# dobraczka/kiez

Hardware: AMD Instinct MI355X
Metric: source queries/sec (fit+kneighbors) + recall@k vs reference, 1/2/4/8 GPU (higher is better)
Workload: dtype f16

## Files before the change

### include/kiez_amd.h

```cpp
#ifndef KIEZ_AMD_H
#define KIEZ_AMD_H

#include <stddef.h>
#include <stdint.h>

#ifdef __cplusplus
extern "C" {
#endif

#define KZ_ABI_VERSION 7
#define KZ_MAX_CANDIDATES 4096
#define KZ_MERGE_MAX_ENTRIES 8192

enum { KZ_OK = 0, KZ_ERR_INVALID = 1, KZ_ERR_HIP = 2, KZ_ERR_UNSUPPORTED = 3, KZ_ERR_NOMEM = 4, KZ_ERR_NONFINITE = 5 };
enum { KZ_F32 = 0, KZ_F64 = 1 };
enum { KZ_EUCLIDEAN = 0, KZ_SQEUCLIDEAN = 1, KZ_COSINE = 2, KZ_MANHATTAN = 3, KZ_CHEBYSHEV = 4, KZ_MINKOWSKI = 5,
       KZ_BRAYCURTIS = 6, KZ_SEUCLIDEAN = 7, KZ_CORRELATION = 8, KZ_HAMMING = 9,
       KZ_JACCARD = 10, KZ_DICE = 11, KZ_ROGERSTANIMOTO = 12, KZ_RUSSELLRAO = 13, KZ_SOKALMICHENER = 14, KZ_SOKALSNEATH = 15,
       KZ_YULE = 16 };

typedef struct kz_ctx kz_ctx;
typedef struct kz_matrix kz_matrix;

typedef struct kz_knn_stats {
// ... 6 lines not shown
    int32_t n_blocks;
    int32_t first_pass;
    int64_t n_escalated_rows;
    double max_err_ratio;
    int32_t dual;
    int32_t n_first_pass_fail;
    int64_t n_events;
    int64_t n_overflow_rows;
    int64_t n_logged_groups;
    int32_t wide_lists;
    int32_t n_spec_rows;
    double probe_ms;
    int64_t n_range_rows;
    int64_t n_range_pairs;
    int64_t n_range_group_rows;
} kz_knn_stats;

int kz_abi_version(void);
const char* kz_last_error(void);
int kz_device_count(int* n);
int kz_ctx_create(int device, void* stream, kz_ctx** out);
int kz_ctx_destroy(kz_ctx* ctx);
int kz_ctx_sync(kz_ctx* ctx);
int kz_ctx_trim(kz_ctx* ctx);
int kz_ctx_set_option(kz_ctx* ctx, const char* name, double value);

int kz_malloc(kz_ctx* ctx, size_t bytes, void** d_ptr);
int kz_free(kz_ctx* ctx, void* d_ptr);
int kz_memcpy_h2d(kz_ctx* ctx, void* d_dst, const void* h_src, size_t bytes);
int kz_memcpy_d2h(kz_ctx* ctx, void* h_dst, const void* d_src, size_t bytes);
// ... 90 lines not shown
```

### kiez_amd/_native.py

```python
from __future__ import annotations

import ctypes as C
import os
import sys
import threading
from pathlib import Path
from typing import Optional, Tuple

import numpy as np

_LIB_NAME = "libkiez_amd.so"
_lib = None
_lock = threading.Lock()

KZ_F32, KZ_F64 = 0, 1
KZ_EUCLIDEAN, KZ_SQEUCLIDEAN, KZ_COSINE, KZ_MANHATTAN, KZ_CHEBYSHEV, KZ_MINKOWSKI = 0, 1, 2, 3, 4, 5
KZ_BRAYCURTIS, KZ_SEUCLIDEAN, KZ_CORRELATION, KZ_HAMMING = 6, 7, 8, 9
KZ_JACCARD, KZ_DICE, KZ_ROGERSTANIMOTO, KZ_RUSSELLRAO, KZ_SOKALMICHENER, KZ_SOKALSNEATH, KZ_YULE = 10, 11, 12, 13, 14, 15, 16
BOOLEAN_METRICS = ("jaccard", "dice", "rogerstanimoto", "russellrao", "sokalmichener", "sokalsneath", "yule")
METRIC_IDS = {"euclidean": KZ_EUCLIDEAN, "sqeuclidean": KZ_SQEUCLIDEAN, "cosine": KZ_COSINE, "manhattan": KZ_MANHATTAN,
              "chebyshev": KZ_CHEBYSHEV, "minkowski": KZ_MINKOWSKI, "braycurtis": KZ_BRAYCURTIS, "seuclidean": KZ_SEUCLIDEAN,
              "correlation": KZ_CORRELATION, "hamming": KZ_HAMMING, "jaccard": KZ_JACCARD, "dice": KZ_DICE,
              "rogerstanimoto": KZ_ROGERSTANIMOTO, "russellrao": KZ_RUSSELLRAO, "sokalmichener": KZ_SOKALMICHENER,
              "sokalsneath": KZ_SOKALSNEATH, "yule": KZ_YULE}
# ... 23 lines not shown
        ("n_blocks", C.c_int32),
        ("first_pass", C.c_int32),
        ("n_escalated_rows", C.c_int64),
        ("max_err_ratio", C.c_double),
        ("dual", C.c_int32),
        ("n_first_pass_fail", C.c_int32),
        ("n_events", C.c_int64),
        ("n_overflow_rows", C.c_int64),
        ("n_logged_groups", C.c_int64),
        ("wide_lists", C.c_int32),
        ("n_spec_rows", C.c_int32),
        ("probe_ms", C.c_double),
        ("n_range_rows", C.c_int64),
        ("n_range_pairs", C.c_int64),
        ("n_range_group_rows", C.c_int64),
    ]

    def as_dict(self):
        return {name: getattr(self, name) for name, _ in self._fields_}


_P = C.c_void_p
_I64 = C.c_int64
SYMBOLS = [
    ("kz_abi_version", C.c_int, []),
    ("kz_last_error", C.c_char_p, []),
    ("kz_device_count", C.c_int, [C.POINTER(C.c_int)]),
    ("kz_ctx_create", C.c_int, [C.c_int, _P, C.POINTER(_P)]),
    ("kz_ctx_destroy", C.c_int, [_P]),
    ("kz_ctx_sync", C.c_int, [_P]),
# ... 375 lines not shown
```

### kiez_amd/csrc/kz_common.h

```cpp
#pragma once
#include <hip/hip_runtime.h>

#include <cstdarg>
#include <cstdint>
#include <cstdio>
#include <cstring>
#include <memory>

#include "../../include/kiez_amd.h"
#include "kz_pool_buf.h"

#define KZ_TILE 128
#define KZ_KSLICE 16
#define KZ_LIVE_MAX 1024
#define KZ_POOL_SLOTS 256

constexpr double KZ_K_NESTED_MIN_MS = 2.0;
constexpr int KZ_K_DUAL_SHORT_DIV = 5;
constexpr int KZ_K_DUAL_SHORT_KP = 16;
constexpr double KZ_K_PROBE_MIN_MS = 12.0;
constexpr int KZ_K_EXACT_DIRECT_ROWS = 32;
constexpr double KZ_K_SPEC_ELEMS = 1.6e9;
constexpr int KZ_K_FLOOR_PROBE = 1024;

struct kz_ctx {
    int device;
    hipStream_t stream;
    bool own_stream;
    hipEvent_t ev[12];
    int stream2_busy;
    hipStream_t stream2;
    double eps_scale;
    int force_splits;
    int chunk_rows;
    int precision;
    int dual_stride;
    int esc_bf;
    int short_ord_min_tiles;
// ... 8 lines not shown
    int dual_force;
    int h_q64;
    int fin_fast_div;
    double probe_min_pairs;
    int list_floor;
    int tier_probe;
    int dual_nested;
    int esc_ladder;
    int exact_rows;
    int abl;
    double floor_margin;
    int dual_rank;
    int spec_rows;
    int wide_lists;
    int wide_sel;
    void* scratch;
    size_t scratch_bytes;
    float* floor_buf;
    size_t floor_bytes;
    int* d_counters;
    int* h_counters;
    int n_cus;
    void* h_stage;
    size_t h_stage_bytes;
    int h_stage_flip;
    struct { void* ptr; size_t bytes; } pool[KZ_POOL_SLOTS];
    int pool_n;
    size_t pool_bytes;
    void* live_ptr[KZ_LIVE_MAX];
    size_t live_bytes[KZ_LIVE_MAX];
// ... 320 lines not shown
```

### kiez_amd/csrc/kz_floor.h

```cpp
#pragma once

static inline bool kz_floor_fit(const double* pairs, int n_probe, double margin_scale, double* model) {
    model[0] = model[1] = model[2] = 0.0;
    if (n_probe <= 0) return false;
    double sx = 0, sy = 0;
    for (int i = 0; i < n_probe; ++i) {
        sx += pairs[2 * i];
        sy += pairs[2 * i + 1];
    }
    const double mx = sx / n_probe, my = sy / n_probe;
    double sxx = 0, sxy = 0;
    for (int i = 0; i < n_probe; ++i) {
        sxx += (pairs[2 * i] - mx) * (pairs[2 * i] - mx);
        sxy += (pairs[2 * i] - mx) * (pairs[2 * i + 1] - my);
    }
    const double beta = sxx > 0 ? sxy / sxx : 0.0, alpha = my - beta * mx;
    double short_max = 0;
    for (int i = 0; i < n_probe; ++i) {
        const double r = alpha + beta * pairs[2 * i] - pairs[2 * i + 1];
        if (r > short_max) short_max = r;
    }
    model[0] = alpha;
    model[1] = beta;
    model[2] = short_max * margin_scale;
    return (alpha - alpha == 0.0) && (beta - beta == 0.0) && (model[2] - model[2] == 0.0);
}
```

### kiez_amd/csrc/kz_knn.hip

```cpp
#include <vector>

#include <algorithm>
#include <atomic>
#include <type_traits>

#include "kz_common.h"
#include "kz_bool.h"
#include "kz_floor.h"

#include "kz_knn_device.h"

template <int KP, int NRES>
__global__ __launch_bounds__(256, 3) void kz_knn_cand_kernel(KnnCandParams p) {
    extern __shared__ __attribute__((aligned(16))) char smem[];
    float* ybuf = reinterpret_cast<float*>(smem);
    const int tid = threadIdx.x;
    const int lane = tid & 63;
    const int wave = tid >> 6;
    const int j = lane & 31;
    const int h = lane >> 5;

    const int4 wd = p.work[blockIdx.x];
    const int qt = wd.x;
    const int t_begin = wd.y;
// ... 348 lines not shown
        return;
    }
    const double qc2 = rowq[r * 3 + 0], qh = rowq[r * 3 + 1], qr = rowq[r * 3 + 2];
    const double Yh = y_hmax[0], Ry = y_hmax[1], Yc2 = y_hmax[2];
    const double qc = sqrt(qc2), yc = sqrt(Yc2);
    const double eps = eps_mult * (qr * Yh + qh * Ry + qr * Ry + gamma_acc * (0.5 * Yc2 + qh * Yh) +
                                   1.1920928955078125e-07 * (qc + yc) * (qc + yc) + 1e-12 * (0.5 * Yc2 + qc2));
    const double f = (alpha + beta * qc2 - margin - eps) / hscale[1];
    float ff = (float)f;
    if ((double)ff > f) ff = nextafterf(ff, -INFINITY);
    out[p] = ff;
}

static inline double kz_gamma_acc_h(int kg) { return 2.0 * (double)(kg * 4 + 16) * 5.9604644775390625e-08; }
static int kz_floor_model(kz_ctx* ctx, const double* dist, const double* rowq, int n_probe, int64_t stride, int k, int metric, double* model,
                          bool* ok) {
    KzPoolBuf<double> d_pairs;
    int rc = d_pairs.alloc(ctx, (size_t)n_probe * 16);
    if (rc != KZ_OK) return rc;
    std::vector<double> hp((size_t)n_probe * 2);
    hipLaunchKernelGGL(kz_floor_pairs_kernel, dim3((unsigned)((n_probe + 255) / 256)), dim3(256), 0, ctx->stream, dist, rowq, n_probe, stride, k,
                       metric, d_pairs.get());
    hipError_t e = hipGetLastError();
    if (e == hipSuccess) e = hipMemcpyAsync(hp.data(), d_pairs.get(), (size_t)n_probe * 16, hipMemcpyDeviceToHost, ctx->stream);
    if (e == hipSuccess) e = hipStreamSynchronize(ctx->stream);
    d_pairs.reset();
    if (e != hipSuccess) {
        kz_set_error("kz_knn: floor probe failed: %s", hipGetErrorString(e));
        return KZ_ERR_HIP;
    }
    *ok = kz_floor_fit(hp.data(), n_probe, ctx->floor_margin, model);
    return KZ_OK;
}

__global__ void kz_boot_floor_kernel(const float* __restrict__ in_key, const int* __restrict__ in_idx, KzListLayout lay, int KP, int64_t list_row0,
                                     int64_t q_begin, int64_t q_count, const float* __restrict__ prev, float* __restrict__ out) {
    const int64_t q = (int64_t)blockIdx.x * blockDim.x + threadIdx.x;
    if (q >= q_count) return;
    const int64_t l0 = kz_list_contig_off(list_row0 + q, lay, KP, 0);
    float mn = INFINITY;
    bool full = true;
    for (int e = 0; e < KP; ++e) {
        full = full && in_idx[l0 + e] >= 0;
        mn = fminf(mn, in_key[l0 + e]);
    }
    float f = full ? mn : -INFINITY;
// ... 120 lines not shown
    KZ_REQUIRE(query->ctx == ctx && index->ctx == ctx, "%s: matrices belong to a different context", who);
    KZ_REQUIRE(!query->raw_only && !index->raw_only, "%s: a rows-only matrix (kz_matrix_create rows_on_device = 3) cannot be searched", who);
    KZ_REQUIRE(query->d == index->d, "%s: feature dimensions differ (%lld vs %lld)", who, (long long)query->d, (long long)index->d);
    KZ_REQUIRE(query->dtype == index->dtype, "%s: query and index must have the same dtype", who);
    KZ_REQUIRE(query->metric == index->metric && query->mink_p == index->mink_p, "%s: query and index were packed for different metrics", who);
    KZ_REQUIRE(kz_metric_params_match(query, index), "%s: seuclidean needs the same V (kz_matrix_set_seuclidean_v) on query and index", who);
    KZ_REQUIRE(q_begin >= 0 && q_count >= 0 && q_begin + q_count <= query->n, "%s: query row range out of bounds", who);
    return KZ_OK;
}

static int kz_knn_impl(kz_ctx* ctx, kz_matrix* query, int64_t q_begin, int64_t q_count, kz_matrix* index, int k,
                       int exclude_self, const int64_t* d_self_ids, KzResearch rs, double* d_dist,
                       int64_t* d_ind, kz_knn_stats* stats, KzDualPass* dual);
static int kz_escalate_rows(kz_ctx* ctx, kz_matrix* query, int64_t cq_begin, const int* fail_list, int n_fail, kz_matrix* index, int k,
                            int exclude_self, const int64_t* d_self_ids, KzResearch rs, double* out_dist,
                            int64_t* out_ind, kz_knn_stats* st2, float* ms_out) {
    KZ_HIP(hipEventRecord(ctx->ev[3], ctx->stream));
    const size_t row_bytes = (size_t)query->d * (query->dtype == KZ_F32 ? 4 : 8);
    KzPoolBuf<int64_t> sub_ind;
    KzPoolBuf<double> sub_dist;
    KzPoolBuf<int64_t> sub_self;
    KzPoolBuf<void> sub_raw;
    KzPoolBuf<int> fl;
    KzMatrixPtr qsub;
    int rc = fl.alloc(ctx, (size_t)n_fail * sizeof(int));
    if (rc == KZ_OK) rc = sub_raw.alloc(ctx, (size_t)n_fail * row_bytes);
    if (rc == KZ_OK && exclude_self) rc = sub_self.alloc(ctx, (size_t)n_fail * 8);
    if (rc == KZ_OK) rc = sub_dist.alloc(ctx, (size_t)n_fail * k * 8);
    if (rc == KZ_OK) rc = sub_ind.alloc(ctx, (size_t)n_fail * k * 8);
    if (rc != KZ_OK) return rc;
    hipError_t e = hipMemcpyAsync(fl.get(), fail_list, (size_t)n_fail * sizeof(int), hipMemcpyDeviceToDevice, ctx->stream);
// ... 2 lines not shown
                           n_fail, (int64_t)row_bytes, (char*)sub_raw.get(), sub_self.get(), d_self_ids);
        e = hipGetLastError();
    }
    if (e != hipSuccess) {
        kz_set_error("kz_knn: gathering the escalated rows failed: %s", hipGetErrorString(e));
        return KZ_ERR_HIP;
    }
    kz_matrix* qsub_new = nullptr;
    rc = kz_matrix_create(ctx, sub_raw.get(), 2, n_fail, query->d, query->dtype, query->metric, &qsub_new);
    qsub.reset(qsub_new);
    memset(st2, 0, sizeof(*st2));
    if (rc == KZ_OK)
        rc = kz_knn_impl(ctx, qsub.get(), 0, n_fail, index, k, exclude_self, sub_self.get(), rs, sub_dist.get(), sub_ind.get(), st2, nullptr);
    if (rc == KZ_OK) {
        hipLaunchKernelGGL(kz_scatter_rows_kernel, dim3((unsigned)(((int64_t)n_fail * k + 255) / 256)), dim3(256), 0, ctx->stream,
                           sub_dist.get(), sub_ind.get(), fl.get(), n_fail, k, out_dist, out_ind);
        e = hipGetLastError();
        if (e == hipSuccess) e = hipEventRecord(ctx->ev[4], ctx->stream);
        if (e == hipSuccess) e = hipStreamSynchronize(ctx->stream);
        if (e != hipSuccess) {
            kz_set_error("kz_knn: scattering the escalated rows failed: %s", hipGetErrorString(e));
            rc = KZ_ERR_HIP;
        }
    }
    if (rc != KZ_OK) return rc;
    KZ_HIP(hipEventElapsedTime(ms_out, ctx->ev[3], ctx->ev[4]));
    return KZ_OK;
}

__global__ void kz_strided_pick_kernel(const int* __restrict__ in, int n_out, int64_t stride, int* __restrict__ out) {
    const int i = blockIdx.x * blockDim.x + threadIdx.x;
// ... 673 lines not shown
```

### kiez_amd/csrc/kz_knn_dual.h

```cpp
#pragma once

constexpr int KZ_EVC = 1;

__global__ __launch_bounds__(256) void kz_dual_theta_kernel(const float* __restrict__ in_key, const int* __restrict__ in_idx,
                                                            KzListLayout lay, int KP, int rank, int64_t n_b, int64_t n_b_pad,
                                                            const float* __restrict__ bias_b, const double* __restrict__ a_hmax,
                                                            const double* __restrict__ b_hmax, const double* __restrict__ hscale,
                                                            float* __restrict__ theta, float* __restrict__ floor_,
                                                            const int* __restrict__ idx_to_row, int sev_cap, int* __restrict__ sev_cnt,
                                                            uint2* __restrict__ sev) {
    const int lane = threadIdx.x & 63;
    const int64_t t = (int64_t)blockIdx.x * 4 + (threadIdx.x >> 6);
    if (t >= n_b_pad) return;
    if (t >= n_b) {
        if (lane == 0) theta[t] = INFINITY;
        return;
    }
    const int M = lay.pieces[kz_list_region(t, lay)] * KP;
    const int64_t l0 = kz_list_contig_off(t, lay, KP, 0);
    float x[4];
    int valid[4];
    unsigned ux[4];
    unsigned all_or = 0u, all_and = 0xffffffffu;
    int nv = 0;
// ... 49 lines not shown
                if (pos < sev_cap) sev[t * (int64_t)sev_cap + pos] = make_uint2(__float_as_uint(x[u]), (unsigned)idx_to_row[in_idx[l0 + lane + 64 * u]]);
            }
            base += (int)__popcll(mask);
        }
        if (lane == 0) sev_cnt[t] = base;
    }
    if (lane == 0) {
        const double S2 = hscale[0] * hscale[0];
        const double margin = 4.76837158203125e-07 * S2 * (a_hmax[0] * b_hmax[0] + a_hmax[2] + b_hmax[2]);
        const double th = (double)tau + (double)bias_b[t] - margin;
        float tf = (float)th;
        if ((double)tf > th) tf = nextafterf(tf, -INFINITY);
        theta[t] = tf;
        floor_[t] = tau_bound;
    }
}

__global__ __launch_bounds__(256) void kz_dual_sample_kernel(const uint4* __restrict__ packed, const float* __restrict__ bias,
                                                             int nsr, int stride, int s_tiles, int P,
                                                             uint4* __restrict__ s_packed, float* __restrict__ s_bias) {
    const int jp = blockIdx.x;
    const int n_frag = 2 * nsr * KZ_TILE;
    for (int e = threadIdx.x; e < n_frag; e += 256) {
        const int row = e & (KZ_TILE - 1), blk = e >> 7;
        const int64_t j = kz_dealt_row((int64_t)jp * KZ_TILE + row, (int64_t)s_tiles * KZ_TILE, P);
        const int64_t src_tile = (j >> 7) * stride;
        s_packed[(int64_t)jp * n_frag + e] = packed[src_tile * n_frag + blk * KZ_TILE + (j & (KZ_TILE - 1))];
        if (blk == 0) s_bias[(int64_t)jp * KZ_TILE + row] = bias[src_tile * KZ_TILE + (j & (KZ_TILE - 1))];
    }
}
// ... 451 lines not shown
        const double img_b = ((double)s_tiles + (double)a_tiles + (double)b_tiles) * (double)n_slices * 4096.0;
        size_t free_b = 0, total_b = 0;
        KZ_HIP(hipMemGetInfo(&free_b, &total_b));
        const double avail = (double)free_b + (double)ctx->pool_bytes - 2.0 * (double)(1ull << 30);
        const double budget = ctx->dual_max_gb > 0 ? ctx->dual_max_gb * (double)(1ull << 30) : KZ_DUAL_MAX_BYTES;
        if (ev_b + log_b + img_b > budget || ev_b + log_b + img_b > avail)
            return kz_knn_dual_separately(ctx, a, b, k, d_dist_ab, d_ind_ab, d_dist_ba, d_ind_ba, stats_ab, stats_ba);
    }

    int rc = kz_himage_ensure(a, b);
    if (rc != KZ_OK) return rc;
    const kz_himage* ia = a->himg;
    const kz_himage* ib = b->himg;
    const int64_t b_pad = b_tiles * KZ_TILE, a_pad = a_tiles * KZ_TILE;

    const int ev_cap = (int)(((int64_t)rank * stride + (int64_t)(7.0 * sqrt((double)rank) * stride) + 63) & ~(int64_t)63);
    const long long log_cap = (long long)((double)b->n * rank * stride * 1.5) + (1 << 20);

    int then = 0, sep_prec = -1, sep_wide = 0;
    kz_knn_stats st_ba;
    memset(&st_ba, 0, sizeof(st_ba));
    const int rc_pass = [&]() -> int {
    KzPoolBuf<unsigned long long> d_cnt;
    KzPoolBuf<void> log_meta, log_keys;
    KzPoolBuf<uint2> ev;
    KzPoolBuf<int> fail_list, col_idx, ev_cnt;
    KzPoolBuf<float> col_key, qfloor, qnb, floor_, theta;
    KzPoolBuf<int> perm, iota;
    KzPoolBuf<float> theta_min, theta_s;
    KzPoolBuf<int> row_map, q_sorted, q_iota;
    KzPoolBuf<float> q_key_s, q_key, q_bias;
    KzPoolBuf<unsigned short> q_packed;
    KzPoolBuf<float> p_bias;
    KzPoolBuf<unsigned short> p_packed;
// ... 26 lines not shown
    if (rc == KZ_OK) rc = q_iota.alloc(ctx, (size_t)a_pad * 4);
    if (rc == KZ_OK) rc = q_sorted.alloc(ctx, (size_t)a_pad * 4);
    if (rc == KZ_OK) rc = row_map.alloc(ctx, (size_t)a_pad * 4);
    if (rc == KZ_OK) rc = p_bias.alloc(ctx, (size_t)b_pad * 4);
    if (rc == KZ_OK) rc = theta_s.alloc(ctx, (size_t)b_pad * 4);
    if (rc == KZ_OK) rc = theta_min.alloc(ctx, (size_t)b_pad * 4);
    if (rc == KZ_OK) rc = iota.alloc(ctx, (size_t)b_pad * 4);
    if (rc == KZ_OK) rc = perm.alloc(ctx, (size_t)b_pad * 4);
    if (rc == KZ_OK) rc = theta.alloc(ctx, (size_t)b_pad * 4);
    if (rc == KZ_OK) rc = floor_.alloc(ctx, (size_t)b_pad * 4);
    if (rc == KZ_OK) rc = qnb.alloc(ctx, (size_t)a_pad * 4);
    if (rc == KZ_OK) rc = col_key.alloc(ctx, (size_t)b->n * KPr * 4);
    if (rc == KZ_OK) rc = col_idx.alloc(ctx, (size_t)b->n * KPr * 4);
    if (rc == KZ_OK) rc = ev_cnt.alloc(ctx, (size_t)b_pad * 4 * KZ_EVC);
    if (rc == KZ_OK) rc = fail_list.alloc(ctx, (size_t)b->n * 4);
    if (rc == KZ_OK) rc = ev.alloc(ctx, (size_t)b_pad * ev_cap * 8);
    if (rc == KZ_OK) rc = log_keys.alloc(ctx, (size_t)log_cap * 16);
    if (rc == KZ_OK) rc = log_meta.alloc(ctx, (size_t)log_cap * 8);
    if (rc == KZ_OK) rc = d_cnt.alloc(ctx, KZ_DUAL_CNT_BYTES);
    if (rc != KZ_OK) {
        then = 1;
        return KZ_OK;
    }
    double floor_model[3] = {0, 0, 0};
    bool have_floor = false;
    bool tier_probed = false;
    bool want_floor = ctx->list_floor && KZ_K_FLOOR_PROBE > 0 && a->n >= (int64_t)16 * KZ_K_FLOOR_PROBE &&
                      (ctx->dual_force || t_sweep_ms >= (KP > 16 ? 12.0 : 25.0));
    const bool want_tier = !ctx->dual_force && ctx->tier_probe > 0 && ctx->esc_bf && a->n >= (int64_t)16 * ctx->tier_probe &&
                           ((double)a->n * (double)b->n >= ctx->probe_min_pairs || t_sweep_ms >= KZ_K_PROBE_MIN_MS);
    if (want_tier && ctx->list_floor && KZ_K_FLOOR_PROBE > 0 && a->n >= (int64_t)16 * KZ_K_FLOOR_PROBE) want_floor = true;
    if (want_floor || want_tier) {
        const int n_probe = want_floor ? KZ_K_FLOOR_PROBE : (ctx->tier_probe < 1024 ? ctx->tier_probe : 1024);
        const int64_t pstride = a->n / n_probe;
        KzPoolBuf<int> plist;
        rc = plist.alloc(ctx, (size_t)n_probe * sizeof(int));
        if (rc == KZ_OK && want_floor) rc = qfloor.alloc(ctx, (size_t)a_pad * 4);
        kz_knn_stats stp;
        memset(&stp, 0, sizeof(stp));
// ... 14 lines not shown
                rc = kz_escalate_rows(ctx, a, 0, plist.get(), n_probe, b, k, 0, nullptr, kz_research_wide(ctx->wide_lists), d_dist_ab, d_ind_ab, &stw,
                                      &wms);
                if (rc == KZ_OK && stw.wide_lists > 0 && (int64_t)stw.n_first_pass_fail * 4 <= n_probe &&
                    (int64_t)stw.n_first_pass_fail * 2 < stp.n_first_pass_fail)
                    wide = ctx->wide_lists;
            }
            if (rc != KZ_OK) return rc;
            if (wide > 0 || (int64_t)stp.n_first_pass_fail * 2 > n_probe) {
                then = 1;
                sep_prec = wide > 0 ? -1 : 2;
                sep_wide = wide;
                return KZ_OK;
            }
        }
        plist.reset();
        if (rc == KZ_OK && want_floor) rc = kz_floor_model(ctx, d_dist_ab, ia->rowq, n_probe, pstride, k, a->metric, floor_model, &have_floor);
        if (rc != KZ_OK) return rc;
        if (!have_floor) qfloor.reset();
    }

    auto sample_lists = [&](int rank_, int64_t tiles_, int* kps_out, int* force_out, int head = 2) {
        int kps = KP, force = 0;
        if (ctx->dual_sample_short && KP > 16) {
            kps = rank_ > 96 ? 32 : 16;
            const int need = (head * rank_ + kps - 1) / kps, cap = 256 / kps;
            force = need < cap ? need : cap;
            if ((int64_t)force * 4 > tiles_ || force * kps < rank_) {
                kps = KP;
                force = 0;
            }
        }
        *kps_out = kps;
        *force_out = force;
// ... 6 lines not shown
    hipLaunchKernelGGL(kz_dual_c2key_kernel, dim3((unsigned)((a->n + 255) / 256)), dim3(256), 0, ctx->stream, ia->rowq, a->n, q_key.get());
    hipLaunchKernelGGL(kz_iota_kernel, dim3((unsigned)((a_pad + 255) / 256)), dim3(256), 0, ctx->stream, q_iota.get(), (int)a_pad);
    KZ_HIP(hipGetLastError());
    rc = kz_sort_pairs_f32_i32(ctx, q_key.get(), q_key_s.get(), q_iota.get(), q_sorted.get(), (int)a->n, 0);
    if (rc != KZ_OK) return rc;
    hipLaunchKernelGGL(kz_dual_deal_kernel, dim3((unsigned)((a_pad + 255) / 256)), dim3(256), 0, ctx->stream, q_sorted.get(), a->n, a_pad, row_map.get());
    KZ_HIP(hipGetLastError());
    rc = kz_himage_pack_permuted(a, row_map.get(), q_packed.get(), q_bias.get());
    if (rc != KZ_OK) return rc;
    hipLaunchKernelGGL(kz_dual_negbias_kernel, dim3((unsigned)((a_pad + 255) / 256)), dim3(256), 0, ctx->stream, q_bias.get(), a->n, a_pad, qnb.get());

    int rank3 = 0, stride3 = 0, KPs3 = KP, force_s3 = 0, ev_cap3 = 0;
    int64_t s3_tiles = 0;
    long long log_cap3 = 0;
    const int64_t s_img_rows = s_tiles * KZ_TILE;
    bool nested = ctx->dual_nested && s_tiles >= 8 && s_tiles < a->n / KZ_TILE && s_img_rows >= (int64_t)8 * KP &&
                  b->n <= kz_rows_per_chunk(ctx, KP, false) && (ctx->dual_force || t_sweep_ms / stride >= KZ_K_NESTED_MIN_MS);
    if (nested) {
        const double t2_ms = 2.0 * (double)b->n * (double)s_img_rows * (double)(a->kg * 4) / 1e12;
        const int rank3_safe = k + 1 < KP ? k + 1 : KP;
        rank3 = rank3_safe;
        if (ctx->dual_rank > 0)
            rank3 = ctx->dual_rank < rank3_safe ? ctx->dual_rank : rank3_safe;
        else if (ctx->dual_rank == 0 && t2_ms >= 4.0)
            rank3 = kz_dual_pick_rank(k, rank3_safe, t2_ms, (double)b->n, (double)s_img_rows);
        const double s_opt = sqrt(t2_ms / ((double)s_img_rows * rank3 * 0.20e-6));
        stride3 = s_opt < 4.0 ? 4 : (s_opt > 32.0 ? 32 : (int)(s_opt + 0.5));
        const int s_max = (int)(4096.0 / ((double)rank3 + 7.0 * sqrt((double)rank3) + 1.0));
        if (stride3 > s_max) stride3 = s_max;
        s3_tiles = (b_tiles + stride3 - 1) / stride3;
        int64_t s3_rows = s3_tiles * KZ_TILE;
        if ((b_tiles - 1) % stride3 == 0) s3_rows -= b_tiles * KZ_TILE - b->n;
// ... 154 lines not shown
            hipLaunchKernelGGL(kz_dual_theta_kernel, dim3((unsigned)((h.b_pad + 3) / 4)), dim3(256), 0, ctx->stream, d2.lists_key, d2.lists_idx,
                               d2.lists_lay, d2.lists_KP, h.rank, h.b_n, h.b_pad, h.ib->bias, h.ia->d_max, h.ib->d_max, h.ib->center->d_scale,
                               h.theta, h.floor_, h.rm3, h.sev_cap, h.sev_cnt, h.sev);
            KZ_HIP(hipGetLastError());
            return kz_dual_enqueue_chain(*h.rv3);
        };
        kz_knn_stats st2;
        ctx->stream2_busy = 1;
        rc = kz_knn_impl(ctx, b, 0, b->n, a, k, 0, nullptr, KzResearch(), d_dist_ba, d_ind_ba, &st2, &dp2);
        if (rc != KZ_OK) return rc;
        if (dp2.broken || !dp2.post_called) {
            then = 1;
            return KZ_OK;
        }
        nested_sweep_ms = st2.main_kernel_ms;
    } else {
        hipLaunchKernelGGL(kz_dual_sample_kernel, dim3((unsigned)s_tiles), dim3(256), 0, ctx->stream, (const uint4*)ia->packed, ia->bias,
                           n_slices, stride, (int)s_tiles, force_s > 0 ? force_s : 1, (uint4*)s_packed.get(), s_bias.get());
        KZ_HIP(hipGetLastError());
        const int KP = KPs;
        int blocks_per_cu = 1;
        KZ_DISPATCH_KP(rc, kz_h_occupancy, (n_slices, &blocks_per_cu));
        if (rc != KZ_OK) return rc;
        KzPass ps;
        const int slots = kz_h_slots(n_slices, blocks_per_cu, ctx->n_cus);
        KzPlan pl;
        kz_plan_tier_pass(ctx, (int)b_tiles, (int)s_tiles, slots, 256 / KP, KP, KZ_TIER_H, 1, force_s, 0, &pl);
        rc = kz_prepare_pass(ctx, pl, (int)s_tiles, slots, KZ_TIER_H, 0, &ps);
        if (rc != KZ_OK) return rc;
        KnnCandParams cp;
// ... 96 lines not shown
    if (rc == KZ_OK && !ctx->dual_overlap && !dp.broken) {
        dp.post_called = 1;
        rc = enqueue_reverse(&rv);
    }
    {
        const hipError_t e2 = hipStreamSynchronize(ctx->stream2);
        ctx->stream2_busy = 0;
        if (rc == KZ_OK && e2 != hipSuccess) {
            kz_set_error("kz_knn_dual: second stream failed: %s", hipGetErrorString(e2));
            rc = KZ_ERR_HIP;
        }
    }
    if (rc != KZ_OK) return rc;
    KZ_HIP(hipEventElapsedTime(&sample_ms, ctx->ev[5], ctx->ev[6]));
    st_ab.dual = 1;
    st_ab.main_kernel_ms += nested_sweep_ms;
    if (nested) {
        int n_fail3 = ctx->h_counters[24];
        unsigned long long hc3[4];
        memcpy(hc3, ctx->h_counters + 28, 32);
        const int* list3 = nst.fail3.get();
        if (hc3[0] > (unsigned long long)log_cap3) {
            n_fail3 = (int)s_img_rows;
            list3 = nst.rm3.get();
        }
        const bool rescued3 = hc3[0] <= (unsigned long long)log_cap3 && spec_s3.R > 0 && n_fail3 > 0 && n_fail3 <= spec_s3.R;
        if (rescued3) {
            st_ab.n_fallback_rows += n_fail3;
            st_ab.n_spec_rows += n_fail3;
        } else if (n_fail3 > 0) {
// ... 10 lines not shown
        double r3;
        memcpy(&r3, ctx->h_counters + 26, 8);
        if (r3 > st_ab.max_err_ratio) st_ab.max_err_ratio = r3;
        st_ab.n_first_pass_fail += n_fail3;
    }
    kz_dual_fill_stats(stats_ab, st_ab);

    if (!dp.broken && !dp.post_called) dp.broken = 1;
    if (!dp.broken) {
        const int n_fail = ctx->h_counters[12];
        unsigned long long hc[4];
        memcpy(hc, ctx->h_counters + 16, 32);
        memcpy(&st_ba.max_err_ratio, ctx->h_counters + 14, 8);
        float ms = 0;
        KZ_HIP(hipEventElapsedTime(&ms, ctx->ev[8], ctx->ev[9]));
        st_ba.main_kernel_ms = sample_ms - (float)nested_sweep_ms + ms;
        KZ_HIP(hipEventElapsedTime(&ms, ctx->ev[9], ctx->ev[10]));
        st_ba.finalize_ms = ms;
        st_ba.list_len = KPr;
        st_ba.n_splits = 1;
        st_ba.first_pass = KZ_TIER_H;
        st_ba.dual = 1;
        st_ba.n_events = (int64_t)hc[1];
        st_ba.n_overflow_rows = (int64_t)hc[2];
        st_ba.n_logged_groups = (int64_t)(hc[0] & ((1ull << 62) - 1));
        if (hc[0] > (unsigned long long)log_cap) {
            dp.broken = 1;
        } else if (spec_ba.R > 0 && n_fail > 0 && n_fail <= spec_ba.R) {
            st_ba.n_fallback_rows = n_fail;
            st_ba.n_spec_rows = n_fail;
        } else if (n_fail > 0) {
// ... 26 lines not shown
```

### kiez_amd/csrc/kz_options.h

```cpp
#pragma once
#include <cstddef>

#include "kz_common.h"

enum { KZ_OPT_INT = 0, KZ_OPT_BOOL = 1, KZ_OPT_F64 = 2 };
enum { KZ_OPT_PUBLIC = 1, KZ_OPT_SET = 2  };

struct KzOption {
    const char* name;
    int kind;
    size_t offset;
    double lo, hi;
    double dflt;
    unsigned flags;
    double allowed[4];
    int n_allowed;
    const char* doc;
};

#define KZ_O(field) offsetof(kz_ctx, field)
static const KzOption KZ_OPTIONS[] = {
    {"precision", KZ_OPT_INT, KZ_O(precision), 0, 2, 0, KZ_OPT_PUBLIC, {}, 0,
     "first-pass operands: 0 fp16 on centred operands (default), 2 split-bf16, 1 float32; the neighbour order is the float64 one either way"},
    {"dual_stride", KZ_OPT_INT, KZ_O(dual_stride), 0, 64, 1, KZ_OPT_PUBLIC, {}, 0,
// ... 16 lines not shown
    {"spec_rows", KZ_OPT_INT, KZ_O(spec_rows), 0, 64, 64, 0, {}, 0, "exact kernels launched speculatively behind every finalize for at most this many uncertified rows (0 = off)"},
    {"wide_lists", KZ_OPT_INT, KZ_O(wide_lists), 2, 32, 32, KZ_OPT_SET, {0}, -1, "fp16 tier's wide route: lists of 16 per query (0 = off)"},
    {"wide_sel", KZ_OPT_INT, KZ_O(wide_sel), 16, 512, 256, 0, {}, 0, "... entries of those lists the finalize kernel selects"},
    {"floor_margin", KZ_OPT_F64, KZ_O(floor_margin), 0, 1e6, 1.3, 0, {}, 0, "seeded lists: the largest shortfall of the probe below the model, times this (0: the model itself -- half of the rows are searched again; test knob)"},
    {"dual_rank", KZ_OPT_INT, KZ_O(dual_rank), -1, 128, 0, 0, {}, 0, "rank of the sample key that becomes a row's event threshold (0 automatic, -1 = k + 1; 1: many rows short of events, test knob)"},
    {"list_floor", KZ_OPT_INT, KZ_O(list_floor), 0, 1, 1, 0, {}, 0, "seeded candidate lists (population floor from a probe)"},
    {"fin_fast_div", KZ_OPT_INT, KZ_O(fin_fast_div), 0, 1, 1, 0, {}, 0, "cosine re-rank through one reciprocal per candidate row (bit-identical)"},
    {"dual_force", KZ_OPT_BOOL, KZ_O(dual_force), 0, 1, 0, 0, {}, 0, "run the shared sweep also where its cost model says it does not pay (tests)"},
    {"dual_overlap", KZ_OPT_BOOL, KZ_O(dual_overlap), 0, 1, 1, 0, {}, 0, "reverse direction's chain on the second stream"},
    {"dual_nested", KZ_OPT_BOOL, KZ_O(dual_nested), 0, 1, 1, 0, {}, 0, "sampled rows are swept by the sample sweep only (itself a shared sweep)"},
    {"dual_rev_long", KZ_OPT_BOOL, KZ_O(dual_rev_long), 0, 1, 1, 0, {}, 0, "reverse lists of twice the list length"},
    {"dual_sample_short", KZ_OPT_BOOL, KZ_O(dual_sample_short), 0, 1, 1, 0, {}, 0, "sample sweep keeps lists of 16 (32) over several ranges"},
    {"dual_short_main", KZ_OPT_BOOL, KZ_O(dual_short_main), 0, 1, 1, 0, {}, 0, "main sweep keeps k / dual_short_div lists of 16 (13 .. 110 neighbours)"},
    {"dual_short_extra", KZ_OPT_INT, KZ_O(dual_short_extra), 1, 200, 48, 0, {}, 0, "entries selected beyond k on that route"},
    {"dual_short_min_tiles", KZ_OPT_INT, KZ_O(dual_short_min_tiles), 1, 1e9, 128, 0, {}, 0, "... taken when an index range has at least this many tiles"},
};
#undef KZ_O
static const int KZ_N_OPTIONS = (int)(sizeof(KZ_OPTIONS) / sizeof(KZ_OPTIONS[0]));

static inline void kz_option_store(kz_ctx* c, const KzOption& o, double v) {
    char* p = reinterpret_cast<char*>(c) + o.offset;
    if (o.kind == KZ_OPT_F64)
        *reinterpret_cast<double*>(p) = v;
    else
        *reinterpret_cast<int*>(p) = o.kind == KZ_OPT_BOOL ? (v != 0 ? 1 : 0) : (int)v;
}
static inline void kz_options_defaults(kz_ctx* c) {
    for (int i = 0; i < KZ_N_OPTIONS; ++i) kz_option_store(c, KZ_OPTIONS[i], KZ_OPTIONS[i].dflt);
}
```

Baseline: 2.650 million.

## Derive dual-sweep event thresholds from a probe regression model instead of a sample sweep

Adds a path in the shared (dual) sweep that probes about 1024 reverse-direction rows exactly. It fits a linear model of each row's k-th neighbour score against its norm and sets per-row event thresholds from that model, replacing the nested or sample sweep. It also sizes the event and log buffers from the model's observed event counts, which can shrink allocations. The path is gated on fit quality (R^2), no saturated or short probe rows, and a memory budget. The cost is an extra probe search and host fit, plus more rows needing re-search if the model's thresholds turn out loose.

```diff
diff --git a/include/kiez_amd.h b/include/kiez_amd.h
--- a/include/kiez_amd.h
+++ b/include/kiez_amd.h
@@ -44,6 +44,10 @@
     int64_t n_range_rows;
     int64_t n_range_pairs;
     int64_t n_range_group_rows;
+    int32_t thresh_source;
+    int32_t model_max_events;
+    double model_mean_events;
+    double floor_r2;
 } kz_knn_stats;
 
 int kz_abi_version(void);
diff --git a/kiez_amd/_native.py b/kiez_amd/_native.py
--- a/kiez_amd/_native.py
+++ b/kiez_amd/_native.py
@@ -61,6 +61,10 @@
         ("n_range_rows", C.c_int64),
         ("n_range_pairs", C.c_int64),
         ("n_range_group_rows", C.c_int64),
+        ("thresh_source", C.c_int32),
+        ("model_max_events", C.c_int32),
+        ("model_mean_events", C.c_double),
+        ("floor_r2", C.c_double),
     ]
 
     def as_dict(self):
diff --git a/kiez_amd/csrc/kz_common.h b/kiez_amd/csrc/kz_common.h
--- a/kiez_amd/csrc/kz_common.h
+++ b/kiez_amd/csrc/kz_common.h
@@ -22,6 +22,7 @@
 constexpr int KZ_K_EXACT_DIRECT_ROWS = 32;
 constexpr double KZ_K_SPEC_ELEMS = 1.6e9;
 constexpr int KZ_K_FLOOR_PROBE = 1024;
+constexpr double KZ_K_MODEL_MIN_R2 = 0.45;
 
 struct kz_ctx {
     int device;
@@ -60,6 +61,8 @@
     int spec_rows;
     int wide_lists;
     int wide_sel;
+    int dual_model;
+    double dual_model_shift;
     void* scratch;
     size_t scratch_bytes;
     float* floor_buf;
diff --git a/kiez_amd/csrc/kz_floor.h b/kiez_amd/csrc/kz_floor.h
--- a/kiez_amd/csrc/kz_floor.h
+++ b/kiez_amd/csrc/kz_floor.h
@@ -1,4 +1,5 @@
 #pragma once
+#include <cstddef>
 
 static inline bool kz_floor_fit(const double* pairs, int n_probe, double margin_scale, double* model) {
     model[0] = model[1] = model[2] = 0.0;
@@ -25,3 +26,69 @@
     model[2] = short_max * margin_scale;
     return (alpha - alpha == 0.0) && (beta - beta == 0.0) && (model[2] - model[2] == 0.0);
 }
+
+static inline double kz_floor_r2(const double* pairs, int n_probe) {
+    if (n_probe < 2) return 0.0;
+    double sx = 0, sy = 0;
+    for (int i = 0; i < n_probe; ++i) {
+        sx += pairs[2 * i];
+        sy += pairs[2 * i + 1];
+    }
+    const double mx = sx / n_probe, my = sy / n_probe;
+    double sxx = 0, sxy = 0, syy = 0;
+    for (int i = 0; i < n_probe; ++i) {
+        const double dx = pairs[2 * i] - mx, dy = pairs[2 * i + 1] - my;
+        sxx += dx * dx;
+        sxy += dx * dy;
+        syy += dy * dy;
+    }
+    if (!(sxx > 0) || !(syy > 0)) return 0.0;
+    const double r2 = sxy * sxy / (sxx * syy);
+    return r2 - r2 == 0.0 ? (r2 < 1.0 ? r2 : 1.0) : 0.0;
+}
+
+struct KzThetaFit {
+    double alpha, beta, margin;
+    double mean_count;
+    int max_count, n_saturated, n_short;
+};
+static inline bool kz_theta_fit(const double* rows, int n_probe, int k_p, int k, double margin_scale, KzThetaFit* out) {
+    out->alpha = out->beta = out->margin = out->mean_count = 0.0;
+    out->max_count = out->n_saturated = out->n_short = 0;
+    if (n_probe <= 0 || k < 1 || k_p < k) return false;
+    const size_t w = (size_t)k_p + 1;
+    double sx = 0, sy = 0;
+    for (int i = 0; i < n_probe; ++i) {
+        sx += rows[i * w];
+        sy += rows[i * w + k];
+    }
+    const double mx = sx / n_probe, my = sy / n_probe;
+    double sxx = 0, sxy = 0;
+    for (int i = 0; i < n_probe; ++i) {
+        sxx += (rows[i * w] - mx) * (rows[i * w] - mx);
+        sxy += (rows[i * w] - mx) * (rows[i * w + k] - my);
+    }
+    const double beta = sxx > 0 ? sxy / sxx : 0.0, alpha = my - beta * mx;
+    double short_max = 0;
+    for (int i = 0; i < n_probe; ++i) {
+        const double r = alpha + beta * rows[i * w] - rows[i * w + k];
+        if (r > short_max) short_max = r;
+    }
+    const double margin = short_max * margin_scale;
+    if (!((alpha - alpha == 0.0) && (beta - beta == 0.0) && (margin - margin == 0.0))) return false;
+    long long total = 0;
+    for (int i = 0; i < n_probe; ++i) {
+        const double tau = alpha + beta * rows[i * w] - margin;
+        int c = 0;
+        for (int j = 1; j <= k_p; ++j) c += rows[i * w + j] >= tau ? 1 : 0;
+        total += c;
+        if (c > out->max_count) out->max_count = c;
+        if (c == k_p) ++out->n_saturated;
+        if (c < k) ++out->n_short;
+    }
+    out->alpha = alpha;
+    out->beta = beta;
+    out->margin = margin;
+    out->mean_count = (double)total / n_probe;
+    return true;
+}
diff --git a/kiez_amd/csrc/kz_knn.hip b/kiez_amd/csrc/kz_knn.hip
--- a/kiez_amd/csrc/kz_knn.hip
+++ b/kiez_amd/csrc/kz_knn.hip
@@ -1,3 +1,4 @@
+#include <chrono>
 #include <vector>
 
 #include <algorithm>
@@ -386,7 +387,7 @@
 
 static inline double kz_gamma_acc_h(int kg) { return 2.0 * (double)(kg * 4 + 16) * 5.9604644775390625e-08; }
 static int kz_floor_model(kz_ctx* ctx, const double* dist, const double* rowq, int n_probe, int64_t stride, int k, int metric, double* model,
-                          bool* ok) {
+                          bool* ok, double* r2 = nullptr) {
     KzPoolBuf<double> d_pairs;
     int rc = d_pairs.alloc(ctx, (size_t)n_probe * 16);
     if (rc != KZ_OK) return rc;
@@ -402,6 +403,7 @@
         return KZ_ERR_HIP;
     }
     *ok = kz_floor_fit(hp.data(), n_probe, ctx->floor_margin, model);
+    if (r2) *r2 = *ok ? kz_floor_r2(hp.data(), n_probe) : 0.0;
     return KZ_OK;
 }
 
@@ -552,7 +554,7 @@
                        int64_t* d_ind, kz_knn_stats* stats, KzDualPass* dual);
 static int kz_escalate_rows(kz_ctx* ctx, kz_matrix* query, int64_t cq_begin, const int* fail_list, int n_fail, kz_matrix* index, int k,
                             int exclude_self, const int64_t* d_self_ids, KzResearch rs, double* out_dist,
-                            int64_t* out_ind, kz_knn_stats* st2, float* ms_out) {
+                            int64_t* out_ind, kz_knn_stats* st2, float* ms_out, const int* out_rows = nullptr) {
     KZ_HIP(hipEventRecord(ctx->ev[3], ctx->stream));
     const size_t row_bytes = (size_t)query->d * (query->dtype == KZ_F32 ? 4 : 8);
     KzPoolBuf<int64_t> sub_ind;
@@ -585,7 +587,7 @@
         rc = kz_knn_impl(ctx, qsub.get(), 0, n_fail, index, k, exclude_self, sub_self.get(), rs, sub_dist.get(), sub_ind.get(), st2, nullptr);
     if (rc == KZ_OK) {
         hipLaunchKernelGGL(kz_scatter_rows_kernel, dim3((unsigned)(((int64_t)n_fail * k + 255) / 256)), dim3(256), 0, ctx->stream,
-                           sub_dist.get(), sub_ind.get(), fl.get(), n_fail, k, out_dist, out_ind);
+                           sub_dist.get(), sub_ind.get(), out_rows ? out_rows : fl.get(), n_fail, k, out_dist, out_ind);
         e = hipGetLastError();
         if (e == hipSuccess) e = hipEventRecord(ctx->ev[4], ctx->stream);
         if (e == hipSuccess) e = hipStreamSynchronize(ctx->stream);
diff --git a/kiez_amd/csrc/kz_knn_dual.h b/kiez_amd/csrc/kz_knn_dual.h
--- a/kiez_amd/csrc/kz_knn_dual.h
+++ b/kiez_amd/csrc/kz_knn_dual.h
@@ -87,6 +87,50 @@
         theta[t] = tf;
         floor_[t] = tau_bound;
     }
+}
+
+__global__ void kz_dual_model_rows_kernel(const double* __restrict__ dist, const double* __restrict__ rowq, int n_probe, int64_t stride, int k_p,
+                                          int metric, double* __restrict__ out) {
+    const int64_t e = (int64_t)blockIdx.x * blockDim.x + threadIdx.x;
+    if (e >= (int64_t)n_probe * (k_p + 1)) return;
+    const int i = (int)(e / (k_p + 1)), j = (int)(e - (int64_t)i * (k_p + 1));
+    const double x = rowq[(int64_t)i * stride * 3];
+    if (j == 0) {
+        out[e] = x;
+        return;
+    }
+    const double v = dist[(int64_t)i * k_p + j - 1];
+    const double d2 = metric == KZ_EUCLIDEAN ? v * v : (metric == KZ_COSINE ? 2.0 * v : v);
+    out[e] = 0.5 * (x - d2);
+}
+__global__ void kz_dual_model_theta_kernel(int64_t n_b, int64_t n_b_pad, const double* __restrict__ rowq_b, const float* __restrict__ bias_b,
+                                           const double* __restrict__ a_hmax, const double* __restrict__ b_hmax,
+                                           const double* __restrict__ hscale, double alpha, double beta, double margin, double eps_mult,
+                                           double gamma_acc, float* __restrict__ theta, float* __restrict__ floor_) {
+    const int64_t t = (int64_t)blockIdx.x * blockDim.x + threadIdx.x;
+    if (t >= n_b_pad) return;
+    if (t >= n_b) {
+        theta[t] = INFINITY;
+        floor_[t] = INFINITY;
+        return;
+    }
+    const double tc2 = rowq_b[t * 3 + 0], th = rowq_b[t * 3 + 1], tr = rowq_b[t * 3 + 2];
+    const double Ah = a_hmax[0], Ra = a_hmax[1], Ac2 = a_hmax[2];
+    const double tc = sqrt(tc2), ac = sqrt(Ac2);
+    const double eps = eps_mult * (tr * Ah + th * Ra + tr * Ra + gamma_acc * (0.5 * Ac2 + th * Ah) +
+                                   1.1920928955078125e-07 * (tc + ac) * (tc + ac) + 1e-12 * (0.5 * Ac2 + tc2));
+    const double f = (alpha + beta * tc2 - margin - eps) / hscale[1];
+    float tau = (float)f;
+    if ((double)tau > f) tau = nextafterf(tau, -INFINITY);
+    if (!(f < (double)INFINITY)) tau = INFINITY;
+    const double S2 = hscale[0] * hscale[0];
+    const double m2 = 4.76837158203125e-07 * S2 * (Ah * b_hmax[0] + Ac2 + b_hmax[2]);
+    const double thd = (double)tau + (double)bias_b[t] - m2;
+    float tf = (float)thd;
+    if ((double)tf > thd) tf = nextafterf(tf, -INFINITY);
+    if (tau == INFINITY) tf = INFINITY;
+    theta[t] = tf;
+    floor_[t] = tau;
 }
 
 __global__ __launch_bounds__(256) void kz_dual_sample_kernel(const uint4* __restrict__ packed, const float* __restrict__ bias,
@@ -568,10 +612,11 @@
     const kz_himage* ib = b->himg;
     const int64_t b_pad = b_tiles * KZ_TILE, a_pad = a_tiles * KZ_TILE;
 
-    const int ev_cap = (int)(((int64_t)rank * stride + (int64_t)(7.0 * sqrt((double)rank) * stride) + 63) & ~(int64_t)63);
-    const long long log_cap = (long long)((double)b->n * rank * stride * 1.5) + (1 << 20);
+    int ev_cap = (int)(((int64_t)rank * stride + (int64_t)(7.0 * sqrt((double)rank) * stride) + 63) & ~(int64_t)63);
+    long long log_cap = (long long)((double)b->n * rank * stride * 1.5) + (1 << 20);
 
     int then = 0, sep_prec = -1, sep_wide = 0;
+    int thresh_source = 0;
     kz_knn_stats st_ba;
     memset(&st_ba, 0, sizeof(st_ba));
     const int rc_pass = [&]() -> int {
@@ -628,15 +673,13 @@
     if (rc == KZ_OK) rc = col_idx.alloc(ctx, (size_t)b->n * KPr * 4);
     if (rc == KZ_OK) rc = ev_cnt.alloc(ctx, (size_t)b_pad * 4 * KZ_EVC);
     if (rc == KZ_OK) rc = fail_list.alloc(ctx, (size_t)b->n * 4);
-    if (rc == KZ_OK) rc = ev.alloc(ctx, (size_t)b_pad * ev_cap * 8);
-    if (rc == KZ_OK) rc = log_keys.alloc(ctx, (size_t)log_cap * 16);
-    if (rc == KZ_OK) rc = log_meta.alloc(ctx, (size_t)log_cap * 8);
     if (rc == KZ_OK) rc = d_cnt.alloc(ctx, KZ_DUAL_CNT_BYTES);
     if (rc != KZ_OK) {
         then = 1;
         return KZ_OK;
     }
     double floor_model[3] = {0, 0, 0};
+    double floor_r2 = 0;
     bool have_floor = false;
     bool tier_probed = false;
     bool want_floor = ctx->list_floor && KZ_K_FLOOR_PROBE > 0 && a->n >= (int64_t)16 * KZ_K_FLOOR_PROBE &&
@@ -681,9 +724,83 @@
             }
         }
         plist.reset();
-        if (rc == KZ_OK && want_floor) rc = kz_floor_model(ctx, d_dist_ab, ia->rowq, n_probe, pstride, k, a->metric, floor_model, &have_floor);
+        if (rc == KZ_OK && want_floor)
+            rc = kz_floor_model(ctx, d_dist_ab, ia->rowq, n_probe, pstride, k, a->metric, floor_model, &have_floor, &floor_r2);
         if (rc != KZ_OK) return rc;
         if (!have_floor) qfloor.reset();
+    }
+
+    const bool nested_sizes = ctx->dual_nested && s_tiles >= 8 && s_tiles < a->n / KZ_TILE && s_tiles * KZ_TILE >= (int64_t)8 * KP &&
+                              b->n <= kz_rows_per_chunk(ctx, KP, false) && (ctx->dual_force || t_sweep_ms / stride >= KZ_K_NESTED_MIN_MS);
+    bool model = false;
+    KzThetaFit mfit;
+    memset(&mfit, 0, sizeof(mfit));
+    float rev_probe_ms = 0;
+    {
+        const bool forced = ctx->dual_model == 2;
+        const int k_cap = 110;
+        int k_p = 6 * k > 64 ? 6 * k : 64;
+        const bool automatic = ctx->dual_model == 1 && !ctx->dual_force && nested_sizes && have_floor && floor_r2 >= KZ_K_MODEL_MIN_R2 &&
+                               b->n >= (int64_t)16 * KZ_K_FLOOR_PROBE && k_p <= k_cap;
+        if (k_p > k_cap) k_p = k_cap;
+        if ((int64_t)k_p > a->n) k_p = (int)a->n;
+        if ((forced || automatic) && KZ_K_FLOOR_PROBE > 0 && k_p >= k) {
+            const int n_probe = b->n < KZ_K_FLOOR_PROBE ? (int)b->n : KZ_K_FLOOR_PROBE;
+            const int64_t pstride = b->n / n_probe;
+            const size_t w = (size_t)k_p + 1;
+            KzPoolBuf<double> fit_rows, pdist;
+            KzPoolBuf<int64_t> pind;
+            KzPoolBuf<int> plist, pout;
+            rc = plist.alloc(ctx, (size_t)n_probe * sizeof(int));
+            if (rc == KZ_OK) rc = pout.alloc(ctx, (size_t)n_probe * sizeof(int));
+            if (rc == KZ_OK) rc = pdist.alloc(ctx, (size_t)n_probe * k_p * 8);
+            if (rc == KZ_OK) rc = pind.alloc(ctx, (size_t)n_probe * k_p * 8);
+            if (rc == KZ_OK) rc = fit_rows.alloc(ctx, (size_t)n_probe * w * 8);
+            if (rc == KZ_ERR_NOMEM) rc = KZ_OK;
+            else if (rc == KZ_OK) {
+                hipLaunchKernelGGL(kz_strided_rows_kernel, dim3((unsigned)((n_probe + 255) / 256)), dim3(256), 0, ctx->stream, plist.get(), n_probe, pstride);
+                hipLaunchKernelGGL(kz_iota_kernel, dim3((unsigned)((n_probe + 255) / 256)), dim3(256), 0, ctx->stream, pout.get(), n_probe);
+                KZ_HIP(hipGetLastError());
+                kz_knn_stats stp;
+                memset(&stp, 0, sizeof(stp));
+                KzResearch probe_rs;
+                probe_rs.prec = 0;
+                float esc_ms = 0;
+                const auto t_probe0 = std::chrono::steady_clock::now();
+                rc = kz_escalate_rows(ctx, b, 0, plist.get(), n_probe, a, k_p, 0, nullptr, probe_rs, pdist.get(), pind.get(), &stp, &esc_ms, pout.get());
+                if (rc != KZ_OK) return rc;
+                std::vector<double> hrows((size_t)n_probe * w);
+                hipLaunchKernelGGL(kz_dual_model_rows_kernel, dim3((unsigned)(((size_t)n_probe * w + 255) / 256)), dim3(256), 0, ctx->stream, pdist.get(),
+                                   ib->rowq, n_probe, pstride, k_p, b->metric, fit_rows.get());
+                KZ_HIP(hipGetLastError());
+                KZ_HIP(hipMemcpyAsync(hrows.data(), fit_rows.get(), hrows.size() * 8, hipMemcpyDeviceToHost, ctx->stream));
+                KZ_HIP(hipStreamSynchronize(ctx->stream));
+                const bool fit_ok = kz_theta_fit(hrows.data(), n_probe, k_p, k, ctx->floor_margin, &mfit);
+                rev_probe_ms = std::chrono::duration<float, std::milli>(std::chrono::steady_clock::now() - t_probe0).count();
+                model = fit_ok && (forced || (mfit.n_saturated == 0 && mfit.n_short == 0 && mfit.mean_count < (double)rank * stride));
+            } else {
+                return rc;
+            }
+        }
+    }
+    if (model) {
+        int64_t cap = ((int64_t)2 * mfit.max_count + 63) & ~(int64_t)63;
+        ev_cap = (int)(cap < 64 ? 64 : (cap > 4096 ? 4096 : cap));
+        log_cap = (long long)(2.0 * (double)b->n * mfit.mean_count) + (1 << 20);
+    }
+    if (model) {
+        const double budget = ctx->dual_max_gb > 0 ? ctx->dual_max_gb * (double)(1ull << 30) : KZ_DUAL_MAX_BYTES;
+        if ((double)b_pad * ev_cap * 8.0 + (double)log_cap * 24.0 > budget) {
+            then = 1;
+            return KZ_OK;
+        }
+    }
+    rc = ev.alloc(ctx, (size_t)b_pad * ev_cap * 8);
+    if (rc == KZ_OK) rc = log_keys.alloc(ctx, (size_t)log_cap * 16);
+    if (rc == KZ_OK) rc = log_meta.alloc(ctx, (size_t)log_cap * 8);
+    if (rc != KZ_OK) {
+        then = 1;
+        return KZ_OK;
     }
 
     auto sample_lists = [&](int rank_, int64_t tiles_, int* kps_out, int* force_out, int head = 2) {
@@ -720,8 +837,7 @@
     int64_t s3_tiles = 0;
     long long log_cap3 = 0;
     const int64_t s_img_rows = s_tiles * KZ_TILE;
-    bool nested = ctx->dual_nested && s_tiles >= 8 && s_tiles < a->n / KZ_TILE && s_img_rows >= (int64_t)8 * KP &&
-                  b->n <= kz_rows_per_chunk(ctx, KP, false) && (ctx->dual_force || t_sweep_ms / stride >= KZ_K_NESTED_MIN_MS);
+    bool nested = nested_sizes && !model;
     if (nested) {
         const double t2_ms = 2.0 * (double)b->n * (double)s_img_rows * (double)(a->kg * 4) / 1e12;
         const int rank3_safe = k + 1 < KP ? k + 1 : KP;
@@ -906,6 +1022,11 @@
             return KZ_OK;
         }
         nested_sweep_ms = st2.main_kernel_ms;
+    } else if (model) {
+        hipLaunchKernelGGL(kz_dual_model_theta_kernel, dim3((unsigned)((b_pad + 255) / 256)), dim3(256), 0, ctx->stream, b->n, b_pad, ib->rowq, ib->bias,
+                           ia->d_max, ib->d_max, ib->center->d_scale, mfit.alpha + ctx->dual_model_shift, mfit.beta, mfit.margin, ctx->eps_scale,
+                           kz_gamma_acc_h(a->kg), theta.get(), floor_.get());
+        KZ_HIP(hipGetLastError());
     } else {
         hipLaunchKernelGGL(kz_dual_sample_kernel, dim3((unsigned)s_tiles), dim3(256), 0, ctx->stream, (const uint4*)ia->packed, ia->bias,
                            n_slices, stride, (int)s_tiles, force_s > 0 ? force_s : 1, (uint4*)s_packed.get(), s_bias.get());
@@ -1032,6 +1153,11 @@
     if (rc != KZ_OK) return rc;
     KZ_HIP(hipEventElapsedTime(&sample_ms, ctx->ev[5], ctx->ev[6]));
     st_ab.dual = 1;
+    thresh_source = model ? 3 : (nested ? 2 : 1);
+    st_ab.thresh_source = thresh_source;
+    st_ab.floor_r2 = floor_r2;
+    st_ab.model_max_events = mfit.max_count;
+    st_ab.model_mean_events = mfit.mean_count;
     st_ab.main_kernel_ms += nested_sweep_ms;
     if (nested) {
         int n_fail3 = ctx->h_counters[24];
@@ -1072,7 +1198,11 @@
         memcpy(&st_ba.max_err_ratio, ctx->h_counters + 14, 8);
         float ms = 0;
         KZ_HIP(hipEventElapsedTime(&ms, ctx->ev[8], ctx->ev[9]));
-        st_ba.main_kernel_ms = sample_ms - (float)nested_sweep_ms + ms;
+        st_ba.probe_ms = rev_probe_ms;
+        st_ba.thresh_source = thresh_source;
+        st_ba.model_max_events = mfit.max_count;
+        st_ba.model_mean_events = mfit.mean_count;
+        st_ba.main_kernel_ms = rev_probe_ms + sample_ms - (float)nested_sweep_ms + ms;
         KZ_HIP(hipEventElapsedTime(&ms, ctx->ev[9], ctx->ev[10]));
         st_ba.finalize_ms = ms;
         st_ba.list_len = KPr;
diff --git a/kiez_amd/csrc/kz_options.h b/kiez_amd/csrc/kz_options.h
--- a/kiez_amd/csrc/kz_options.h
+++ b/kiez_amd/csrc/kz_options.h
@@ -54,6 +54,8 @@
     {"dual_short_main", KZ_OPT_BOOL, KZ_O(dual_short_main), 0, 1, 1, 0, {}, 0, "main sweep keeps k / dual_short_div lists of 16 (13 .. 110 neighbours)"},
     {"dual_short_extra", KZ_OPT_INT, KZ_O(dual_short_extra), 1, 200, 48, 0, {}, 0, "entries selected beyond k on that route"},
     {"dual_short_min_tiles", KZ_OPT_INT, KZ_O(dual_short_min_tiles), 1, 1e9, 128, 0, {}, 0, "... taken when an index range has at least this many tiles"},
+    {"dual_model", KZ_OPT_INT, KZ_O(dual_model), 0, 2, 1, 0, {}, 0, "event thresholds from a probe model instead of a sample sweep: 0 never, 1 where the gate allows, 2 forced (tests)"},
+    {"dual_model_shift", KZ_OPT_F64, KZ_O(dual_model_shift), -1e300, 1e300, 0, 0, {}, 0, "... added to the model's thresholds (test knob: a huge value leaves no events, every row is searched again)"},
 };
 #undef KZ_O
 static const int KZ_N_OPTIONS = (int)(sizeof(KZ_OPTIONS) / sizeof(KZ_OPTIONS[0]));
```

New measurement: 2.785 million (median of 6 runs). 1.05x the previous value.
